# baycom/tfrec

Hardware: AMD Instinct MI355X
Metric: IQ MSamples/s through demod+decode (batched streams) (higher is better)
Workload: dtype int32+f32+f64

## Files before the change

include/tfrec_amd.h:

```cpp
#ifndef TFREC_AMD_H
#define TFREC_AMD_H

#include <stddef.h>
#include <stdint.h>

#ifdef __cplusplus
extern "C" {
#endif

#define TFREC_AMD_BLOCK_BYTES 65536
#define TFREC_AMD_FIFO_DEPTH 4
#define TFREC_AMD_BLOCK_BYTES_10X 655360
#define TFREC_AMD_BLOCK_DEC 8192
#define TFREC_AMD_NSLOTS 5

enum { TFREC_AMD_SLOT_TFA1 = 0, TFREC_AMD_SLOT_TFA2 = 1, TFREC_AMD_SLOT_TFA3 = 2, TFREC_AMD_SLOT_TX22 = 3,
       TFREC_AMD_SLOT_WHB = 4 };

enum {
	TFREC_AMD_OK = 0,
	TFREC_AMD_E_INVAL = -1,
	TFREC_AMD_E_NOMEM = -2,
	TFREC_AMD_E_HIP = -3,
	TFREC_AMD_E_OVERFLOW = -4,
// ... 263 lines not shown
	uint64_t floor;
	uint32_t n_hit;
	uint32_t n_frames;
} tfrec_amd_occupancy;
int tfrec_amd_enable_occupancy(tfrec_amd_ctx *ctx, uint32_t ratio, uint32_t rel);
int tfrec_amd_read_occupancy(tfrec_amd_ctx *ctx, int32_t row, tfrec_amd_occupancy *recs, uint32_t *bitmap, size_t cap_records,
			     int *n_records);

int tfrec_amd_rssi_db(int slot, int64_t rssi_raw);

int tfrec_amd_read_stage0(tfrec_amd_ctx *ctx, int stream, int16_t *out, size_t n_pairs);
int tfrec_amd_read_decimated(tfrec_amd_ctx *ctx, int stream, int16_t *out, size_t n_pairs);
typedef struct {
	uint64_t resolved;
	uint64_t host_verified;
	uint64_t host_mismatch;
	uint64_t undecidable;
	uint64_t reserved[4];
} tfrec_amd_fm_stats;
int tfrec_amd_get_fm_stats(tfrec_amd_ctx *ctx, tfrec_amd_fm_stats *out);
int tfrec_amd_atan_uncertain(tfrec_amd_ctx *ctx, uint64_t *n);
int tfrec_amd_fm_dev_probe(int device, int kind, const void *records, size_t n, int32_t *out, tfrec_amd_fm_stats *stats);
int tfrec_amd_iir_probe(int device, double cutoff, int form, const double *in, size_t n, double *out);
int tfrec_amd_read_biquad_row(tfrec_amd_ctx *ctx, int slot, int stream, int32_t *out, size_t cap_values, uint32_t *n_slots);
int tfrec_amd_get_timings(tfrec_amd_ctx *ctx, tfrec_amd_timings *out);
typedef struct {
	uint64_t biquad_segments;
	uint64_t biquad_unconverged;
	uint64_t biquad_serial;
	uint64_t tfa2_resliced;
	uint64_t tfa1_recomputed;
	uint64_t biquad_repair_slots;
	uint64_t whb_respeculated;
	uint64_t tfa1_scalar_groups;
	uint64_t tfa2_scalar_groups;
	uint64_t tfa1_vector_groups;
	uint64_t tfa2_vector_groups;
} tfrec_amd_stats;
int tfrec_amd_get_stats(tfrec_amd_ctx *ctx, tfrec_amd_stats *out);
int tfrec_amd_get_layout(tfrec_amd_ctx *ctx, int *n_streams);
int tfrec_amd_get_memory(tfrec_amd_ctx *ctx, uint64_t *device_bytes, uint64_t *pinned_host_bytes);
int tfrec_amd_read_thresh(tfrec_amd_ctx *ctx, int stream, int *thresh);

#ifdef __cplusplus
}
#endif
// ... 2 lines not shown
```

tfrec_amd/api.py:

```python
from __future__ import annotations

import ctypes as C
import os
from fractions import Fraction

import numpy as np

from . import _build
from .burst import BURST_DTYPE
from .capture import RUN_DTYPE
from .clock import CLOCK_DTYPE
from .envelope import ENVELOPE_DTYPE
from .levels import LEVEL_DTYPE
from .occupancy import OCC_DTYPE
from .sync import SYNC_DTYPE
from .track import TRACK_DTYPE

BLOCK_BYTES = 65536
BLOCK_DEC = 8192
NSLOTS = 5
FIFO_DEPTH = 4
SLOT_NAMES = ("TFA_1", "TFA_2", "TFA_3", "TX22", "WHB")

F_ALL_FLUSHES = 1
# ... 64 lines not shown
    ]
)
assert EVENT_DTYPE.itemsize == 96

EXPORTS = (
    "tfrec_amd_version", "tfrec_amd_strerror", "tfrec_amd_last_error", "tfrec_amd_create", "tfrec_amd_destroy",
    "tfrec_amd_submit_device", "tfrec_amd_submit_host", "tfrec_amd_sync", "tfrec_amd_drain_events",
    "tfrec_amd_pending_events", "tfrec_amd_rssi_db", "tfrec_amd_read_decimated", "tfrec_amd_atan_uncertain",
    "tfrec_amd_get_timings", "tfrec_amd_read_thresh", "tfrec_amd_get_stats", "tfrec_amd_get_layout", "tfrec_amd_host_alloc",
    "tfrec_amd_host_free", "tfrec_amd_read_stage0", "tfrec_amd_get_fm_stats", "tfrec_amd_fm_dev_probe",
    "tfrec_amd_fifo_depth", "tfrec_amd_get_memory", "tfrec_amd_iir_probe", "tfrec_amd_reset_streams",
    "tfrec_amd_configure_streams", "tfrec_amd_get_stream_config", "tfrec_amd_tune_streams", "tfrec_amd_get_stream_tune",
    "tfrec_amd_map_streams", "tfrec_amd_get_stream_input", "tfrec_amd_tune_streams_wide", "tfrec_amd_get_stream_tune_wide",
    "tfrec_amd_create_rate", "tfrec_amd_get_input_rate", "tfrec_amd_input_bytes", "tfrec_amd_resample_taps",
    "tfrec_amd_tune_streams_input", "tfrec_amd_get_stream_tune_input", "tfrec_amd_create_format", "tfrec_amd_get_input_format",
    "tfrec_amd_read_levels", "tfrec_amd_enable_capture", "tfrec_amd_read_captures", "tfrec_amd_enable_spectrum",
    "tfrec_amd_read_spectrum", "tfrec_amd_enable_occupancy", "tfrec_amd_read_occupancy", "tfrec_amd_create_dc", "tfrec_amd_get_dc",
    "tfrec_amd_read_dc", "tfrec_amd_reset_dc_rows", "tfrec_amd_create_iq", "tfrec_amd_get_iq", "tfrec_amd_read_iq", "tfrec_amd_reset_iq_rows", "tfrec_amd_create_decimated", "tfrec_amd_enable_capture_pre",
    "tfrec_amd_read_capture_pre", "tfrec_amd_enable_runs_input", "tfrec_amd_submit_runs", "tfrec_amd_read_biquad_row",
    "tfrec_amd_enable_burst_meter", "tfrec_amd_read_bursts", "tfrec_amd_stream_state_bytes", "tfrec_amd_save_streams",
    "tfrec_amd_load_streams", "tfrec_amd_enable_burst_envelope", "tfrec_amd_read_burst_envelopes",
    "tfrec_amd_enable_burst_clock", "tfrec_amd_read_burst_clocks",
    "tfrec_amd_enable_burst_track", "tfrec_amd_set_burst_track_centre", "tfrec_amd_read_burst_tracks",
    "tfrec_amd_enable_burst_sync", "tfrec_amd_read_burst_syncs",
)

_libs = {}


def library_path(experiments: bool = False, short_segments: bool = False) -> str:
    return _build.VARIANTS[_build.variant_name(experiments, short_segments)][0]


def load_library(build: bool = True, experiments: bool = False, short_segments: bool = False):
    key = _build.variant_name(experiments, short_segments)
    if key in _libs:
        return _libs[key]
    if build:
        try:
            _build.build_device_lib(experiments=bool(experiments), short_segments=bool(short_segments))
        except (OSError, FileNotFoundError):
            pass
    lib_so = library_path(experiments, short_segments)
    if key == "experiments":
        lib_so = os.environ.get("TFREC_AMD_LIB", lib_so)
    if not os.path.exists(lib_so):
        raise RuntimeError("HIP extension %s is missing: run __graft_entry__.build()" % lib_so)
# ... 7 lines not shown
    L.tfrec_amd_strerror.argtypes = [C.c_int]
    L.tfrec_amd_last_error.restype = C.c_char_p
    L.tfrec_amd_create.argtypes = [C.POINTER(Config), C.POINTER(C.c_void_p)]
    L.tfrec_amd_destroy.argtypes = [C.c_void_p]
    L.tfrec_amd_submit_device.argtypes = [C.c_void_p, C.c_void_p, C.c_size_t, C.c_int, C.c_void_p]
    L.tfrec_amd_submit_host.argtypes = [C.c_void_p, C.c_void_p, C.c_size_t, C.c_int]
    L.tfrec_amd_sync.argtypes = [C.c_void_p]
    L.tfrec_amd_drain_events.argtypes = [C.c_void_p, C.c_void_p, C.c_int, C.POINTER(C.c_int)]
    L.tfrec_amd_pending_events.argtypes = [C.c_void_p, C.POINTER(C.c_int)]
    L.tfrec_amd_rssi_db.argtypes = [C.c_int, C.c_int64]
    L.tfrec_amd_rssi_db.restype = C.c_int
    L.tfrec_amd_read_decimated.argtypes = [C.c_void_p, C.c_int, C.c_void_p, C.c_size_t]
    L.tfrec_amd_read_stage0.argtypes = [C.c_void_p, C.c_int, C.c_void_p, C.c_size_t]
    L.tfrec_amd_read_biquad_row.argtypes = [C.c_void_p, C.c_int, C.c_int, C.c_void_p, C.c_size_t, C.POINTER(C.c_uint32)]
    L.tfrec_amd_atan_uncertain.argtypes = [C.c_void_p, C.POINTER(C.c_uint64)]
    L.tfrec_amd_get_timings.argtypes = [C.c_void_p, C.POINTER(Timings)]
    L.tfrec_amd_read_thresh.argtypes = [C.c_void_p, C.c_int, C.POINTER(C.c_int)]
    L.tfrec_amd_get_stats.argtypes = [C.c_void_p, C.POINTER(Stats)]
    L.tfrec_amd_get_layout.argtypes = [C.c_void_p, C.POINTER(C.c_int)]
    L.tfrec_amd_get_memory.argtypes = [C.c_void_p, C.POINTER(C.c_uint64), C.POINTER(C.c_uint64)]
    L.tfrec_amd_get_fm_stats.argtypes = [C.c_void_p, C.POINTER(FmStats)]
    L.tfrec_amd_fm_dev_probe.argtypes = [C.c_int, C.c_int, C.c_void_p, C.c_size_t, C.c_void_p, C.POINTER(FmStats)]
    L.tfrec_amd_iir_probe.argtypes = [C.c_int, C.c_double, C.c_int, C.c_void_p, C.c_size_t, C.c_void_p]
    L.tfrec_amd_reset_streams.argtypes = [C.c_void_p, C.c_void_p, C.c_int]
    L.tfrec_amd_configure_streams.argtypes = [C.c_void_p, C.c_void_p, C.c_void_p, C.c_int]
    L.tfrec_amd_get_stream_config.argtypes = [C.c_void_p, C.c_int, C.POINTER(StreamConfig)]
    L.tfrec_amd_tune_streams.argtypes = [C.c_void_p, C.c_void_p, C.c_void_p, C.c_int]
    L.tfrec_amd_get_stream_tune.argtypes = [C.c_void_p, C.c_int, C.POINTER(C.c_int32)]
    L.tfrec_amd_map_streams.argtypes = [C.c_void_p, C.c_void_p, C.c_void_p, C.c_int]
    L.tfrec_amd_get_stream_input.argtypes = [C.c_void_p, C.c_int, C.POINTER(C.c_int32)]
    L.tfrec_amd_tune_streams_wide.argtypes = [C.c_void_p, C.c_void_p, C.c_void_p, C.c_int]
    L.tfrec_amd_get_stream_tune_wide.argtypes = [C.c_void_p, C.c_int, C.POINTER(C.c_int32)]
    L.tfrec_amd_tune_streams_input.argtypes = [C.c_void_p, C.c_void_p, C.c_void_p, C.c_int]
    L.tfrec_amd_get_stream_tune_input.argtypes = [C.c_void_p, C.c_int, C.POINTER(C.c_int32)]
    L.tfrec_amd_create_rate.argtypes = [C.POINTER(Config), C.c_int32, C.c_int32, C.POINTER(C.c_void_p)]
    L.tfrec_amd_get_input_rate.argtypes = [C.c_void_p, C.POINTER(C.c_int32), C.POINTER(C.c_int32)]
    L.tfrec_amd_input_bytes.argtypes = [C.c_void_p, C.c_int, C.POINTER(C.c_size_t)]
    L.tfrec_amd_resample_taps.argtypes = [C.c_int32, C.c_int32, C.c_void_p, C.c_int, C.POINTER(C.c_int)]
    L.tfrec_amd_create_format.argtypes = [C.POINTER(Config), C.c_int32, C.c_int32, C.c_int32, C.POINTER(C.c_void_p)]
    L.tfrec_amd_get_input_format.argtypes = [C.c_void_p, C.POINTER(C.c_int32)]
    L.tfrec_amd_read_levels.argtypes = [C.c_void_p, C.c_void_p, C.c_size_t, C.POINTER(C.c_int)]
    L.tfrec_amd_enable_capture.argtypes = [C.c_void_p, C.c_uint32, C.c_uint64]
    L.tfrec_amd_read_captures.argtypes = [C.c_void_p, C.c_void_p, C.c_size_t, C.POINTER(C.c_uint32), C.c_void_p, C.c_size_t,
                                          C.POINTER(C.c_uint64)]
    L.tfrec_amd_enable_spectrum.argtypes = [C.c_void_p, C.c_int32, C.c_int32, C.c_int32]
    L.tfrec_amd_read_spectrum.argtypes = [C.c_void_p, C.c_int32, C.c_void_p, C.c_void_p, C.c_size_t, C.c_void_p, C.POINTER(C.c_int)]
# ... 575 lines not shown

    def stats(self) -> dict:
        st = Stats()
        _check(self.L, self.L.tfrec_amd_get_stats(self.h, C.byref(st)))
        return {n: int(getattr(st, n)) for n, _ in Stats._fields_}


def fm_dev_nrzs_probe(records: np.ndarray, device: int = 0) -> np.ndarray:
    L = load_library()
    q = np.ascontiguousarray(records, dtype=np.int32).reshape(-1, 4)
    out = np.empty(len(q), dtype=np.int32)
    _check(L, L.tfrec_amd_fm_dev_probe(device, 2, q.ctypes.data, len(q), out.ctypes.data, None))
    return out


def iir_probe(cutoff: float, x: np.ndarray, form: int = 1, device: int = 0) -> np.ndarray:
    L = load_library()
    xin = np.ascontiguousarray(x, dtype=np.float64)
    out = np.empty(len(xin), dtype=np.float64)
    _check(L, L.tfrec_amd_iir_probe(device, float(cutoff), int(form), xin.ctypes.data, len(xin), out.ctypes.data))
    return out


def fm_dev_probe(records: np.ndarray, device: int = 0, cross: bool = False):
    L = load_library()
    q = (np.ascontiguousarray(records, dtype=np.int64).reshape(-1, 2) if cross
         else np.ascontiguousarray(records, dtype=np.int32).reshape(-1, 4))
    out = np.empty(len(q), dtype=np.int32)
    st = FmStats()
    _check(L, L.tfrec_amd_fm_dev_probe(device, 1 if cross else 0, q.ctypes.data, len(q), out.ctypes.data, C.byref(st)))
    return out, {n: int(getattr(st, n)) for n, _ in FmStats._fields_[:4]}


def events_canon(events: np.ndarray):
    L = load_library()
    events = events[events["status"] != STATUS_BITS]
    m = np.empty((len(events), 71), dtype=np.int64)
    m[:, 0] = events["slot"]
    m[:, 1] = events["end_sample"]
    m[:, 2] = events["byte_cnt"]
    slots = events["slot"].tolist()
    raws = events["rssi_raw"].tolist()
    m[:, 3] = [L.tfrec_amd_rssi_db(sl, rw) for sl, rw in zip(slots, raws)]
    m[:, 4] = events["offset"]
    m[:, 5:69] = events["rdata"]
    m[:, 69] = events["rssi_raw"]
# ... 39 lines not shown
```

tfrec_amd/csrc/capi_create.h:

```cpp
#pragma once

static BiquadCoef biquad_coef(double cutoff)
{
	static const struct {
		double cutoff, b0, a1, a2;
	} known[] = {
		{ 0.5 / (384000.0 / 17240), 0x1.27f98b1037a14p-8, 0x1.cd1527f4a26e2p+0, -0x1.a36a1c41c6995p-1 },
		{ 0.5 / (384000.0 / 9600), 0x1.7ed02b18a270dp-10, 0x1.e397ac010fc89p+0, -0x1.ca2cf85850d62p-1 },
		{ 0.5 / (384000.0 / 8842), 0x1.461fa1a309718p-10, 0x1.e5d4f47377e30p+0, -0x1.ce36282a35d90p-1 },
		{ 2.0 / 64.0, 0x1.14a67102a1ffdp-7, 0x1.b949652fa3970p+0, -0x1.83dd316f714e0p-1 },
		{ 0.0025 / 64.0, 0x1.02ae4cfc8910ap-26, 0x1.ffe9409fe171bp+0, -0x1.ffd283451f7d3p-1 },
	};
	BiquadCoef c;
	for (const auto &k : known)
		if (k.cutoff == cutoff) {
			c.b0 = k.b0;
			c.b1 = k.b0 + k.b0;
			c.b2 = k.b0;
			c.a1 = k.a1;
			c.a2 = k.a2;
			return c;
		}
	const double i = 1.0 / tan(cutoff * M_PI);
	const double s = sqrt(2.0);
// ... 511 lines not shown
		TRY(own_device(c, c->lev.d_records[k], n * (size_t)c->cfg.max_blocks * sizeof(tfrec_amd_level)));
	return make_side_lane(c, c->lev.lane);
}

static int make_streams(tfrec_amd_ctx *c, PipeCtl &S)
{
	int prio_lo = 0, prio_hi = 0;
	(void)hipDeviceGetStreamPriorityRange(&prio_lo, &prio_hi);
	hipStream_t cp = nullptr;
	TRY(own_stream(c, S.fs, prio_hi));
	TRY(own_stream(c, cp, 0));
	TRY(own_stream(c, S.cs, prio_hi));
	S.ws = S.fs;
	c->cpy = cp;
	if (c->cfg.flags & TFREC_AMD_F_SERIAL_CHAINS)
		return TFREC_AMD_OK;
	TRY(own_stream(c, S.t1, prio_hi));
	TRY(own_stream(c, S.aux, prio_hi));
	const char *dp = TFREC_KNOB_STR("DEEP");
	c->deep = dp ? atoi(dp) != 0 : true;
	c->fmdev_k2 = has_kind(c->launch, 1) && has_kind(c->launch, 2);
	S.k2 = S.cs;
	S.kw = S.aux;
	S.vx = S.aux;
	if (!c->deep)
		return TFREC_AMD_OK;
	TRY(own_stream(c, S.k2, 0));
	TRY(own_stream(c, S.kw, 0));
	S.ws = S.kw;
	if (c->fmdev_k2) {
		TRY(own_stream(c, S.fq, prio_lo));
		TRY(own_stream(c, S.ks, prio_lo));
	}
	TRY(own_stream(c, c->cpy, prio_lo));
	S.vx = cp;
	return TFREC_AMD_OK;
}

static int make_pipes(tfrec_amd_ctx *c, const PipeCtl &S)
{
	const bool serial = (c->cfg.flags & TFREC_AMD_F_SERIAL_CHAINS) != 0;
	const bool timing = (c->cfg.flags & TFREC_AMD_F_TIMING) != 0;
	for (int k = 0; k < kSets; k++) {
		PipeCtl &P = c->pipe[k];
		P = S;
		for (hipEvent_t *e : { &P.done[0], &P.done[1], &P.done[2], &P.ev_win, &P.ev_fork, &P.ev_k2, &P.ev_kw, &P.ev_fm,
				       &P.ev_spec, &c->ev_in[k], &P.ev_front, &c->copied[k] })
			TRY(own_event(c, *e, hipEventDisableTiming));
		if (!serial)
			TRY(own_event(c, P.ev_aux, hipEventDisableTiming));
		if (timing) {
			for (hipEvent_t &e : c->ev[k])
				TRY(own_event(c, e, hipEventDefault));
			if (!serial) {
				for (hipEvent_t &e : c->tev[k])
					TRY(own_event(c, e, hipEventDefault));
				P.tev = c->tev[k];
			}
		}
		P.whb_carry = c->d_whbcarry;
		P.fmdev_wmax = c->fmdev_k2 ? c->wmax : 0;
		P.fm_flag_eps = c->fm_flag_eps;
	}
	return TFREC_AMD_OK;
}

static int init_context(tfrec_amd_ctx *c)
{
	if (const char *fe = TFREC_KNOB_STR("FM_FLAG_EPS"))
		c->fm_flag_eps = std::max(1e-9, atof(fe));
	if (const char *cg = TFREC_KNOB_STR("COPY_GUESS_MIN"))
		c->copy_guess = c->copy_guess_min = (uint32_t)std::max(1, atoi(cg));
	TRY(register_chains(c));
// ... 157 lines not shown
```

tfrec_amd/csrc/capi_probe.h:

```cpp
#pragma once

static void account_fm_log(FmTotals *t, const EventBuf &eb)
{
	t->resolved += eb.uncertain;
	t->undecidable += eb.fm_undecidable;
	const uint32_t n = std::min<uint32_t>(eb.fm_logged, (uint32_t)kFmLogCap);
	const double scale = 16384.0 * (1.0 / M_PI);
	for (uint32_t k = 0; k < n; k++) {
		const int want = d2i_host(atan2(eb.fm_log[k].cj, eb.fm_log[k].cr) * scale);
		t->verified++;
		if (want != eb.fm_log[k].result)
			t->mismatch++;
	}
}

static void report_debug_stats(tfrec_amd_ctx *c, int set, int n_blocks)
{
#ifdef TFREC_AMD_VECSTAT
	if (c->submit_seq == 3) {
		(void)hipDeviceSynchronize();
		unsigned long long st[16] = { 0 };
		(void)hipMemcpy(st, c->win[set].stats, sizeof(st), hipMemcpyDeviceToHost);
		fprintf(stderr, "VECSTAT (one submit) TFA_1: groups %llu, stale piece %llu, entered-with-none hazard %llu, > 64 bits in a lane %llu, lanes with 32 ones or more %llu; TFA_2 family: groups %llu, entered with relative 0 %llu, > 16 rounds %llu, > 64 bits in a lane %llu, walks of the groups that converged %llu\n", st[8], st[9], st[10], st[11], st[5], st[12], st[13], st[14], st[15], st[6]);
	}
// ... 199 lines not shown
		stats->undecidable = tmp.undecidable;
	}
	return rc;
}

int tfrec_amd_iir_probe(int device, double cutoff, int form, const double *in, size_t n, double *out)
{
	if (!in || !out || n == 0 || n > (1u << 24) || form < 0 || form > 1 || !(cutoff > 0.0 && cutoff < 0.5))
		return TFREC_AMD_E_INVAL;
	HIPCHK(hipSetDevice(device));
	double *d_in = nullptr, *d_out = nullptr;
	int rc = TFREC_AMD_OK;
	if (hipMalloc((void **)&d_in, n * 8) != hipSuccess || hipMalloc((void **)&d_out, n * 8) != hipSuccess)
		rc = TFREC_AMD_E_NOMEM;
	if (rc == TFREC_AMD_OK && (hipMemcpy(d_in, in, n * 8, hipMemcpyHostToDevice) != hipSuccess ||
				   launch_iir_probe(nullptr, d_in, n, biquad_coef(cutoff), d_out, form) != hipSuccess ||
				   hipMemcpy(out, d_out, n * 8, hipMemcpyDeviceToHost) != hipSuccess))
		rc = hip_fail(hipGetLastError(), "iir_probe");
	(void)hipFree(d_in);
	(void)hipFree(d_out);
	return rc;
}

int tfrec_amd_read_thresh(tfrec_amd_ctx *c, int stream, int *thresh)
{
	if (!c || !thresh || stream < 0 || stream >= c->cfg.n_streams)
		return TFREC_AMD_E_INVAL;
	if (!c->settings.per_stream && c->cfg.thresh) {
		*thresh = c->cfg.thresh;
		return TFREC_AMD_OK;
	}
	TRY(tfrec_amd_sync(c));
	FskState f;
	HIPCHK(hipMemcpy(&f, c->d_fsk + stream, sizeof(f), hipMemcpyDeviceToHost));
	*thresh = f.thresh;
	return TFREC_AMD_OK;
}

int tfrec_amd_get_timings(tfrec_amd_ctx *c, tfrec_amd_timings *out)
{
	if (!c || !out)
		return TFREC_AMD_E_INVAL;
	if (!c->timed)
		return TFREC_AMD_E_STATE;
	const int set = c->last_drained >= 0 ? c->last_drained : c->head;
	hipEvent_t *ev = c->ev[set], *tev = c->tev[set];
// ... 109 lines not shown
```

tfrec_amd/csrc/chains2.hip:

```cpp
#include <stdlib.h>

#include <algorithm>

#include "decoder_dev.h"
#include "launch.h"
#include <type_traits>
#include "whb_chain_asm.h"

namespace tfrec {

constexpr int kSpecLbi = -(1 << 30);

__device__ __forceinline__ int whb_hook_perturb(const WinTables &T)
{
#ifdef TFREC_AMD_EXPERIMENTS
	return T.whb_test_perturb;
#else
	return 0;
#endif
}
__device__ __forceinline__ int whb_hook_force_fail(const WinTables &T)
{
#ifdef TFREC_AMD_EXPERIMENTS
	return T.whb_force_fail;
// ... 158 lines not shown
				const dim3 wgrid(n_streams), wblock(64);
				const int wlds = 64 * 64;
				if (flags & TFREC_AMD_F_BITS) {
					hipLaunchKernelGGL((whb_demod_kernel<true, false>), wgrid, wblock, wlds, P.aux, dec, dec_stride, dev32, n_streams,
							   n_blocks, sample_base, L, a, T, events, eb, flags);
				} else {
					hipLaunchKernelGGL((whb_demod_kernel<false, false>), wgrid, wblock, wlds, P.aux, dec, dec_stride, dev32, n_streams,
							   n_blocks, sample_base, L, a, T, events, eb, flags);
					whb_spec = a;
				}
				mark(kMarkWhbDemodEnd, P.aux);
				mark(kMarkWhbDecodeEnd, P.aux);
				mark(kMarkWhbCommitEnd, P.aux);
			}
	}
	if (whb_spec >= 0) {
		if (P.vx != P.aux) {
			TRY(hipEventRecord(P.ev_aux, P.aux));
			TRY(hipStreamWaitEvent(P.vx, P.ev_aux, 0));
		}
		mark(kMarkWhbCheck, P.vx);
		hipLaunchKernelGGL(whb_chain_kernel, dim3((n_streams + kChkStreams - 1) / kChkStreams), dim3(64 * (1 + kChkProducers)), kChkLdsBytes,
				   P.vx, n_streams, L, whb_spec, T);
		hipLaunchKernelGGL(whb_check_kernel, dim3(n_streams), block, 0, P.vx, n_streams, L, whb_spec, T, P.whb_carry);
		ChainLaunch Lr = L;
		WinTables Tr = T;
		Tr.whbpub = L.states[whb_spec];
		Lr.states[whb_spec] = T.whbscr;
		hipLaunchKernelGGL((whb_demod_kernel<true, true>), dim3((n_streams + 63) / 64), block, 64 * 64, P.vx, dec, dec_stride, dev32, n_streams,
				   n_blocks, sample_base, Lr, whb_spec, Tr, events, eb, flags);
		mark(kMarkWhbCheckEnd, P.vx);
		TRY(hipEventRecord(P.done[1], P.vx));
	} else {
		TRY(hipEventRecord(P.done[1], P.aux));
	}
	static_assert(kMarkTfa2End == kMarkTfa2Coop + 3 && kMarkTfa1End == kMarkTfa1Coop + 3, "a slicer chain's marks are consecutive");
	auto slicer_chain = [&](int kind, hipStream_t s_, int m0) {
		if (kind == 0)
			hipLaunchKernelGGL(mark_kernel, dim3(std::max(1, win_blocks / 16)), dim3(256), 0, s_, dec, dec_stride, n_streams,
					   n_blocks, L, T);
		const size_t slds = (kind == 0 ? 8 : 4) * 64 * sizeof(uint4);
		hipLaunchKernelGGL(slicer_kernel, dim3(std::max(64, win_blocks)), block, slds, s_, dec, dec_stride, ld16, n_streams, n_blocks, L, T,
				   lanes, head_chunks, kind, 0);
		mark(m0, s_);
		hipLaunchKernelGGL(coop_slicer_kernel, dim3(coop_blocks), block, 0, s_, dec, dec_stride, ld16, n_streams, n_blocks, L,
				   T, kind);
		mark(m0 + 1, s_);
		hipLaunchKernelGGL(decode_kernel, dim3(dec_blocks), block, 0, s_, n_streams, L, T, kind);
		mark(m0 + 2, s_);
		hipLaunchKernelGGL(commit_kernel, grid, block, 0, s_, dec, dec_stride, ld16, n_streams, n_blocks, sample_base, L, T,
				   events, eb, flags, lanes, kind);
		if (kind == 1)
			hipLaunchKernelGGL(commit_wave_kernel, dim3(256), block, 0, s_, dec, dec_stride, ld16, n_streams, n_blocks,
					   sample_base, L, T, events, eb, flags);
		mark(m0 + 3, s_);
// ... 40 lines not shown
		TRY(hipEventRecord(P.ev_k2, P.k2));
		TRY(hipStreamWaitEvent(P.cs, P.ev_k2, 0));
		mark(kMarkTfa2Slicer, P.cs);
		slicer_chain(1, P.cs, kMarkTfa2Coop);
	}
	TRY(hipEventRecord(P.done[0], P.cs));
	if (has_tfa1) {
		if (!has_tfa2)
			TRY(hipStreamWaitEvent(P.t1, P.ev_win, 0));
		mark(kMarkTfa1Slicer, P.t1);
		slicer_chain(0, P.t1, kMarkTfa1Coop);
	}
	TRY(hipEventRecord(P.done[2], P.t1));
#undef TRY
	return hipGetLastError();
}

hipError_t whb_chain_lds_optin()
{
	return hipFuncSetAttribute(reinterpret_cast<const void *>(&whb_chain_kernel), hipFuncAttributeMaxDynamicSharedMemorySize,
				   (int)kChkLdsBytes);
}

}
```

tfrec_amd/csrc/launch.h:

```cpp
#pragma once

namespace tfrec {

struct FrontOut {
	uint32_t *dec;             size_t dec_stride;
	unsigned long long *mask;  size_t mask_stride;
	uint32_t *prevdec;
	int16_t *fmdev;            size_t fmdev_stride;
	int n_streams, n_blocks;
};
struct History {
	const uint8_t *in;
	uint8_t *out;
};
struct RateTable {
	int p, q, t;
	const float *taps;
};
struct CaptureBufs {
	CaptureState *state;
	CaptureStage *stage;
	int stage_cap;
	uint2 *cnt;
	uint4 *base;
// ... 45 lines not shown
			   const FrontTapsCfg &taps, bool in16, const uint2 *tune, const uint4 *chan);
hipError_t launch_decin(hipStream_t st, const uint8_t *in, size_t stride, const uint4 *chan, const FrontOut &o, uint32_t *last, int thresh,
			const StreamCfg *scfg);
hipError_t launch_decin_runs(hipStream_t st, const RunsTables &r, const FrontOut &o, uint32_t *last, int thresh, const StreamCfg *scfg);
hipError_t launch_fmdev(hipStream_t st, const FrontOut &o, EventBuf *eb, int wmax, double flag_eps);
hipError_t launch_levels(hipStream_t st, const FrontOut &o, LevelState *lev, const StreamCfg *scfg, tfrec_amd_level *out);
hipError_t launch_capture(hipStream_t st, const FrontOut &o, long long sample_base, const CaptureBufs &b, const StreamCfg *scfg);
hipError_t launch_capture_pre(hipStream_t st, const FrontOut &o, long long sample_base, const CaptureBufs &b, uint32_t *pre);
hipError_t launch_burst_meter(hipStream_t st, const FrontOut &o, const CaptureBufs &b, tfrec_amd_burst *out);
hipError_t launch_burst_envelope(hipStream_t st, const FrontOut &o, const CaptureBufs &b, tfrec_amd_envelope *out);
hipError_t launch_burst_clock(hipStream_t st, const FrontOut &o, const CaptureBufs &b, tfrec_amd_clock *out);
hipError_t launch_burst_track(hipStream_t st, const FrontOut &o, const CaptureBufs &b, const TrackBufs &k);
hipError_t launch_burst_sync(hipStream_t st, const FrontOut &o, const CaptureBufs &b, const SyncBufs &k);
hipError_t launch_spectrum(hipStream_t st, int fmt, const uint8_t *iq, size_t stride, const SpectrumBufs &b);
hipError_t launch_occupancy(hipStream_t st, const SpectrumBufs &b, uint32_t ratio, uint32_t rel, tfrec_amd_occupancy *recs, uint32_t *bits);
hipError_t launch_fm_probe(hipStream_t st, const int32_t *quads, size_t n, int32_t *out, EventBuf *eb, int kind);
hipError_t launch_iir_probe(hipStream_t st, const double *in, size_t n, const BiquadCoef &c, double *out, int form);
hipError_t launch_chains(hipStream_t st, const FrontOut &o, long long sample_base, const ChainLaunch &L, tfrec_amd_event *events,
			 EventBuf *eb, uint32_t flags);
hipError_t launch_threshold(hipStream_t st, const FrontOut &o, FskState *fsk, int wmax, const StreamCfg *scfg);
hipError_t launch_pipeline(const PipeCtl &P, const FrontOut &o, long long sample_base, const ChainLaunch &L, const WinTables &T, int16_t *ld16,
			   int32_t *dev32, tfrec_amd_event *events, EventBuf *eb, uint32_t flags);
hipError_t whb_chain_lds_optin();
struct StateTable;
hipError_t launch_stream_state(hipStream_t st, bool load, const StateTable &T, const int32_t *list, int n_list, uint8_t *stage);

}
```

tfrec_amd/csrc/tfrec_dev.h:

```cpp
#pragma once

#include <hip/hip_runtime.h>
#include <stddef.h>
#include <stdint.h>

#include "../../include/tfrec_amd.h"

#if defined(__HIP_DEVICE_COMPILE__)
#if !defined(__gfx950__)
#error "tfrec_amd: the device code targets gfx950 (MI355X) only"
#endif
#if defined(__AMDGCN_WAVEFRONT_SIZE) && __AMDGCN_WAVEFRONT_SIZE != 64
#error "tfrec_amd: the device code assumes 64-lane wavefronts"
#endif
#endif

namespace tfrec {

constexpr int kBlockDec = TFREC_AMD_BLOCK_DEC;
constexpr int kIndexSpan = 2 * kBlockDec;
constexpr int kTailBytes = 112;
constexpr int kNSlots = TFREC_AMD_NSLOTS;
constexpr int kFmtU8 = TFREC_AMD_FMT_U8, kFmtS8 = TFREC_AMD_FMT_S8, kFmtS16 = TFREC_AMD_FMT_S16, kFmtF32 = TFREC_AMD_FMT_F32;
constexpr int kFmtDec16 = TFREC_AMD_FMT_DEC16;
// ... 291 lines not shown
	int32_t *whbdense;
	int32_t whbdense_stride;
	int32_t *whbdense_n;
	unsigned long long *whbxbits;
	double2 *whbxsnap;
	int32_t whbx_stride;
	int32_t whb_force_fail;
	int32_t whb_submit_seq;
	ChainState *whbscr;
	ChainState *whbpub;
	int32_t whb_test_perturb;
	int32_t tfa2_vec;
	int32_t tfa1_vec;
};
constexpr int kStatusDead = 0xff;

struct PipeCtl {
	hipStream_t fs;
	hipStream_t ws;
	hipEvent_t ev_front;
	hipStream_t k2, kw;
	hipStream_t cs, aux, t1;
	hipStream_t vx;
	hipEvent_t ev_aux;
	int *whb_carry;
	hipEvent_t ev_win;
	hipEvent_t ev_fork;
	hipEvent_t ev_k2, ev_kw;
	hipEvent_t ev_fm;
	hipStream_t fq;
	hipStream_t ks;
	hipEvent_t ev_spec;
	hipEvent_t done[3];
	hipEvent_t *tev;
	int fmdev_wmax;
	double fm_flag_eps;
};
enum TimingMark : int {
	kMarkWindows = 0,
	kMarkTfa2Spec = 1, kMarkTfa2Repair = 2, kMarkTfa2Fix = 3, kMarkTfa2BiquadEnd = 4,
	kMarkTfa2Coop = 5, kMarkTfa2Decode = 6, kMarkTfa2Commit = 7, kMarkTfa2End = 8,
	kMarkWhbSpec = 9, kMarkWhbRepair = 10, kMarkWhbFix = 11, kMarkWhbBiquadEnd = 12,
	kMarkWhbDemodEnd = 13, kMarkWhbDecodeEnd = 14, kMarkWhbCommitEnd = 15,
	kMarkTfa1Slicer = 16, kMarkTfa1Coop = 17, kMarkTfa1Decode = 18, kMarkTfa1Commit = 19, kMarkTfa1End = 20,
	kMarkWindowsEnd = 21, kMarkWhbDemod = 22, kMarkTfa2Slicer = 23, kMarkFmdev = 24, kMarkFmdevEnd = 25,
	kMarkWhbCheck = 26, kMarkWhbCheckEnd = 27,
	kTimingMarks = 28
// ... 27 lines not shown
```

tfrec_amd/csrc/whb_check.h:

```cpp
#pragma once

#ifndef TFREC_AMD_CHK_STREAMS
#define TFREC_AMD_CHK_STREAMS 32
#endif
constexpr int kChkStreams = TFREC_AMD_CHK_STREAMS;
constexpr int kChkProducers = 2;
constexpr int kChkPerProducer = kChkStreams / kChkProducers;
static_assert(kChkStreams <= 64 && kChkStreams % kChkProducers == 0, "a lane per stream, the streams split evenly");
constexpr int kChkPairRow = 64 * 4 + 4;
constexpr int kChkDevRow = 64 + 4;
struct ChkBuf {
	uint32_t pair[kChkStreams * kChkPairRow];
	uint32_t dev[kChkStreams * kChkDevRow];
};
constexpr size_t kChkLdsBytes = 2 * sizeof(ChkBuf);

__global__ __launch_bounds__(64 * (1 + kChkProducers)) void whb_chain_kernel(int n_streams, ChainLaunch L, int a, WinTables T)
{
	extern __shared__ __attribute__((aligned(16))) uint8_t chk_lds[];
	ChkBuf *const buf = reinterpret_cast<ChkBuf *>(chk_lds);
	const int wave = (int)threadIdx.x >> 6, ln = (int)threadIdx.x & 63;
	const int s0 = (int)blockIdx.x * kChkStreams;
	const ChainParams &p = L.params[a];
	const double a1 = p.iir_avg.a1, a2 = p.iir_avg.a2, bh = 0.5 * p.iir_avg.b0;
	const int my_s = s0 + ln;
	const bool my_on = ln < kChkStreams && my_s < n_streams;
	const int my_rounds = my_on ? T.whbdense_n[my_s] >> 6 : 0;
	int rmax = my_rounds;
#pragma unroll
	for (int o = 32; o >= 1; o >>= 1) {
		const int other = __shfl_xor(rmax, o, 64);
		rmax = other > rmax ? other : rmax;
	}
	rmax = __builtin_amdgcn_readfirstlane(rmax);
	if (rmax == 0)
		return;
	if (wave == 0) {
		double y1 = 0.0, y2 = 0.0;
		if (my_on) {
			const WhbExact st = T.whbx[my_s];
			y1 = st.y1;
			y2 = st.y2;
		}
		unsigned long long *const xbits = T.whbxbits + (size_t)(my_on ? my_s : 0) * T.whbx_stride;
		double2 *const xsnap = T.whbxsnap + (size_t)(my_on ? my_s : 0) * T.whbx_stride;
		__syncthreads();
		for (int r = 0; r < rmax; r++) {
			if (r < my_rounds) {
				const ChkBuf &b = buf[r & 1];
				const double2 *prow = reinterpret_cast<const double2 *>(b.pair + ln * kChkPairRow);
				const uint4 *drow = reinterpret_cast<const uint4 *>(b.dev + ln * kChkDevRow);
				uint32_t acc[2] = { 0u, 0u };
				double2 pq[2][8];
				uint4 dq[2][2];
				auto fetch = [&](int h, int g8) {
#pragma unroll
					for (int j = 0; j < 8; j++)
						pq[h][j] = prow[8 * g8 + j];
					dq[h][0] = drow[2 * g8];
					dq[h][1] = drow[2 * g8 + 1];
				};
				fetch(0, 0);
#pragma unroll
				for (int g8 = 0; g8 < 8; g8++) {
					const int h = g8 & 1;
					if (g8 + 1 < 8)
						fetch(h ^ 1, g8 + 1);
					const int dv[8] = { (int)dq[h][0].x, (int)dq[h][0].y, (int)dq[h][0].z, (int)dq[h][0].w,
							    (int)dq[h][1].x, (int)dq[h][1].y, (int)dq[h][1].z, (int)dq[h][1].w };
#pragma unroll
					for (int j = 0; j < 8; j++) {
						const double P = pq[h][j].x, B2 = pq[h][j].y;
						const double y = ((B2 + a1 * y1) + P) + a2 * y2;
						y2 = y1;
						y1 = y;
						const int yi = (int)y;
						asm("v_cmp_lt_i32 vcc, %1, %2\n\tv_addc_co_u32 %0, vcc, %0, %0, vcc" : "+v"(acc[g8 >> 2]) : "v"(dv[j]), "v"(yi) : "vcc");
					}
				}
				xbits[r] = (unsigned long long)__brev(acc[0]) | ((unsigned long long)__brev(acc[1]) << 32);
				xsnap[r] = make_double2(y1, y2);
			}
			__syncthreads();
		}
	} else {
		const int q0 = (wave - 1) * kChkPerProducer;
		int rounds[kChkPerProducer], h1[kChkPerProducer], h2[kChkPerProducer];
		const int32_t *row[kChkPerProducer];
#pragma unroll
		for (int q = 0; q < kChkPerProducer; q++) {
			const int s = s0 + q0 + q;
			const bool on = s < n_streams;
			rounds[q] = __builtin_amdgcn_readlane(my_rounds, (q0 + q) & 63);
			row[q] = T.whbdense + (size_t)(on ? s : 0) * T.whbdense_stride;
			const WhbExact st = T.whbx[on ? s : 0];
			h1[q] = __builtin_amdgcn_readfirstlane(st.fd1);
			h2[q] = __builtin_amdgcn_readfirstlane(st.fd2);
		}
		int cur[kChkPerProducer], nxt[kChkPerProducer];
#pragma unroll
		for (int q = 0; q < kChkPerProducer; q++) {
			cur[q] = rounds[q] > 0 ? row[q][ln] : 0;
			nxt[q] = rounds[q] > 1 ? row[q][64 + ln] : 0;
		}
		auto lay_out = [&](ChkBuf &b, int r) {
#pragma unroll
			for (int q = 0; q < kChkPerProducer; q++) {
				if (r < rounds[q]) {
					const int d0 = cur[q];
					const int s1 = __builtin_amdgcn_update_dpp(0, d0, 0x138, 0xf, 0xf, false);
					const int d1 = ln == 0 ? h1[q] : s1;
					const int s2 = __builtin_amdgcn_update_dpp(0, d1, 0x138, 0xf, 0xf, false);
					const int d2 = ln == 0 ? h2[q] : s2;
					const double t0 = bh * (double)d0, t1 = bh * (double)d1, t2 = bh * (double)d2;
					const double P = __builtin_fma(2.0, t1, t0);
					*reinterpret_cast<double2 *>(b.pair + (q0 + q) * kChkPairRow + 4 * ln) = make_double2(P, t2);
					b.dev[(q0 + q) * kChkDevRow + ln] = (uint32_t)d0;
					h1[q] = __builtin_amdgcn_readlane(d0, 63);
					h2[q] = __builtin_amdgcn_readlane(d0, 62);
				}
			}
		};
		lay_out(buf[0], 0);
		__syncthreads();
		for (int r = 0; r < rmax; r++) {
			int far[kChkPerProducer];
#pragma unroll
			for (int q = 0; q < kChkPerProducer; q++)
				far[q] = r + 2 < rounds[q] ? row[q][64 * (r + 2) + ln] : 0;
#pragma unroll
			for (int q = 0; q < kChkPerProducer; q++)
				cur[q] = nxt[q];
			if (r + 1 < rmax)
				lay_out(buf[(r + 1) & 1], r + 1);
#pragma unroll
			for (int q = 0; q < kChkPerProducer; q++)
				nxt[q] = far[q];
			__syncthreads();
		}
	}
}

constexpr int kChkLockCap = 256;
__global__ __launch_bounds__(64) void whb_check_kernel(int n_streams, ChainLaunch L, int a, WinTables T, int *__restrict__ carry_io)
{
	__shared__ int lk_pos[kChkLockCap], lk_avgf[kChkLockCap];
	__shared__ uint32_t lk_meta[kChkLockCap];
	const int s = (int)blockIdx.x, ln = (int)threadIdx.x;
	if (s >= n_streams)
		return;
	const ChainParams &p = L.params[a];
	const double a1 = p.iir_avg.a1, a2 = p.iir_avg.a2, bh = 0.5 * p.iir_avg.b0;
	const int N = T.whbdense_n[s], R = N >> 6;
	const int32_t *dense = T.whbdense + (size_t)s * T.whbdense_stride;
	const unsigned long long *xbits = T.whbxbits + (size_t)s * T.whbx_stride;
	const double2 *xsnap = T.whbxsnap + (size_t)s * T.whbx_stride;
	const WhbExact st0 = T.whbx[s];
	const int tp_ = whb_hook_perturb(T);
	const int tol = tp_ > 1 ? tp_ : (tp_ < -1 ? -tp_ : 1);
	auto input = [&](int pos) -> int { return pos >= 0 ? dense[pos] : (pos == -1 ? st0.fd1 : st0.fd2); };
	auto run = [&](int rr, int cnt, double &y1, double &y2, unsigned long long &bits) {
		const int p0 = 64 * rr;
		if (rr == 0) {
			y1 = st0.y1;
			y2 = st0.y2;
		} else {
			const double2 sn = xsnap[rr - 1];
			y1 = sn.x;
			y2 = sn.y;
		}
		double t1 = bh * (double)input(p0 - 1), t2 = bh * (double)input(p0 - 2);
		bits = 0ull;
		for (int k = 0; k < cnt; k++) {
			const int d = dense[p0 + k];
			const double t0 = bh * (double)d;
			const double P = __builtin_fma(2.0, t1, t0);
			const double y = ((t2 + a1 * y1) + P) + a2 * y2;
			bits |= (unsigned long long)(d < (int)y ? 1u : 0u) << k;
			y2 = y1;
			y1 = y;
			t2 = t1;
			t1 = t0;
		}
	};
	double yf1 = 0.0, yf2 = 0.0;
	unsigned long long tailbits = 0ull;
	if (ln == 0)
		run(R, N & 63, yf1, yf2, tailbits);
	tailbits = __shfl(tailbits, 0, 64);
	auto word = [&](int i) -> unsigned long long { return i < R ? xbits[i] : (i == R ? tailbits : 0ull); };
	const uint4 *recrow = reinterpret_cast<const uint4 *>(T.whbrec + (size_t)s * T.whbrec_stride);
	int carry = carry_io[s];
	const int carry_in = carry;
	bool bad = false;
	int cbase = 0, nlocks = 0;
	bool ended = false;
	int last_delta = 0;
	bool have_last = false, last_closed = false;
	auto do_locks = [&]() {
		for (int b0 = 0; b0 < nlocks; b0 += 64) {
			const int i = b0 + ln;
			const bool on = i < nlocks;
			double y1 = 0.0, y2 = 0.0;
			unsigned long long bits;
			const int pos = on ? lk_pos[i] : 0;
			run(pos >> 6, on ? (pos & 63) + 1 : 0, y1, y2, bits);
			const uint32_t meta = on ? lk_meta[i] : 0u;
			const int delta = (int)y1 - (on ? lk_avgf[i] : 0);
			const bool b = on && (delta > tol || delta < -tol || (delta != 0 && (meta & kWhbRecAmb)));
			bad = bad || __ballot(b) != 0ull;
			const int nb = nlocks - b0 < 64 ? nlocks - b0 : 64;
			last_delta = __shfl(delta, nb - 1, 64);
			last_closed = (__shfl((int)meta, nb - 1, 64) & (int)kWhbRecClosed) != 0;
// ... 38 lines not shown
		}
		carry = __shfl(carry, 0, 64);
		const bool lock = normal && (meta & kWhbRecLock) != 0u;
		const unsigned long long lm = __ballot(lock);
		if (lm) {
			if (nlocks + 64 > kChkLockCap)
				do_locks();
			if (lock) {
				const int i = nlocks + __builtin_popcountll(lm & ((1ull << ln) - 1ull));
				lk_pos[i] = pos0 + nv - 1;
				lk_avgf[i] = (int)rec.w;
				lk_meta[i] = meta;
			}
			nlocks += __builtin_popcountll(lm);
			__syncthreads();
		}
	}
	if (nlocks)
		do_locks();
	bad = __ballot(bad) != 0ull || cbase != N;
	if (have_last)
		carry = last_closed ? 0 : last_delta;
	if (ln == 0) {
		WhbExact st = st0;
		st.carry = carry_in;
		st.pad_ = 0;
		T.whbx0[s] = st;
		bad = bad || T.whbseen[s] != T.whbgen[s];
		if (whb_hook_force_fail(T) > 0 && (s + T.whb_submit_seq) % whb_hook_force_fail(T) == 0)
			bad = true;
		st.y1 = yf1;
		st.y2 = yf2;
		st.fd1 = input(N - 1);
		st.fd2 = input(N - 2);
		st.carry = st.pad_ = 0;
		T.whbx[s] = st;
		carry_io[s] = bad ? 0 : carry;
		T.whbfail[s] = bad ? 1 : 0;
	}
}
```

Baseline: 305,000.

## Move WHB tail round into chain kernel and run check on separate stream

The chain kernel now also processes the partial tail round of each stream's dense input and writes the final state and the start snapshot (whbx0). This removes the serial single-lane tail recurrence from the check kernel. The check and demod kernels are launched on a new low-priority stream that waits on an event recorded after the chain kernel, so they can overlap with other work in deep mode. A standalone probe API for the chain kernel is added for testing. The risks are the extra event sync and the chain kernel no longer returning early when no stream has a full round.

```diff
diff --git a/include/tfrec_amd.h b/include/tfrec_amd.h
--- a/include/tfrec_amd.h
+++ b/include/tfrec_amd.h
@@ -309,6 +309,13 @@
 int tfrec_amd_atan_uncertain(tfrec_amd_ctx *ctx, uint64_t *n);
 int tfrec_amd_fm_dev_probe(int device, int kind, const void *records, size_t n, int32_t *out, tfrec_amd_fm_stats *stats);
 int tfrec_amd_iir_probe(int device, double cutoff, int form, const double *in, size_t n, double *out);
+typedef struct {
+	double y1, y2;
+	int32_t fd1, fd2;
+	int32_t reserved[2];
+} tfrec_amd_whb_state;
+int tfrec_amd_whb_chain_probe(int device, int n_streams, const int32_t *in, size_t stride, const int32_t *n, tfrec_amd_whb_state *state,
+			      tfrec_amd_whb_state *start, uint64_t *bits, double *snaps);
 int tfrec_amd_read_biquad_row(tfrec_amd_ctx *ctx, int slot, int stream, int32_t *out, size_t cap_values, uint32_t *n_slots);
 int tfrec_amd_get_timings(tfrec_amd_ctx *ctx, tfrec_amd_timings *out);
 typedef struct {
diff --git a/tfrec_amd/api.py b/tfrec_amd/api.py
--- a/tfrec_amd/api.py
+++ b/tfrec_amd/api.py
@@ -110,7 +110,7 @@
     "tfrec_amd_load_streams", "tfrec_amd_enable_burst_envelope", "tfrec_amd_read_burst_envelopes",
     "tfrec_amd_enable_burst_clock", "tfrec_amd_read_burst_clocks",
     "tfrec_amd_enable_burst_track", "tfrec_amd_set_burst_track_centre", "tfrec_amd_read_burst_tracks",
-    "tfrec_amd_enable_burst_sync", "tfrec_amd_read_burst_syncs",
+    "tfrec_amd_enable_burst_sync", "tfrec_amd_read_burst_syncs", "tfrec_amd_whb_chain_probe",
 )
 
 _libs = {}
@@ -164,6 +164,8 @@
     L.tfrec_amd_get_fm_stats.argtypes = [C.c_void_p, C.POINTER(FmStats)]
     L.tfrec_amd_fm_dev_probe.argtypes = [C.c_int, C.c_int, C.c_void_p, C.c_size_t, C.c_void_p, C.POINTER(FmStats)]
     L.tfrec_amd_iir_probe.argtypes = [C.c_int, C.c_double, C.c_int, C.c_void_p, C.c_size_t, C.c_void_p]
+    L.tfrec_amd_whb_chain_probe.argtypes = [C.c_int, C.c_int, C.c_void_p, C.c_size_t, C.c_void_p, C.c_void_p, C.c_void_p, C.c_void_p,
+                                            C.c_void_p]
     L.tfrec_amd_reset_streams.argtypes = [C.c_void_p, C.c_void_p, C.c_int]
     L.tfrec_amd_configure_streams.argtypes = [C.c_void_p, C.c_void_p, C.c_void_p, C.c_int]
     L.tfrec_amd_get_stream_config.argtypes = [C.c_void_p, C.c_int, C.POINTER(StreamConfig)]
@@ -785,6 +787,26 @@
     return out
 
 
+WHB_STATE_DTYPE = np.dtype([("y1", "<f8"), ("y2", "<f8"), ("fd1", "<i4"), ("fd2", "<i4"), ("reserved", "<i4", (2,))])
+assert WHB_STATE_DTYPE.itemsize == 32
+
+
+def whb_chain_probe(rows: np.ndarray, n: np.ndarray, state: np.ndarray, device: int = 0):
+    L = load_library()
+    x = np.ascontiguousarray(rows, dtype=np.int32)
+    ns, stride = x.shape
+    cnt = np.ascontiguousarray(n, dtype=np.int32)
+    end = np.array(state, dtype=WHB_STATE_DTYPE)
+    assert cnt.shape == (ns,) and end.shape == (ns,)
+    start = np.empty(ns, dtype=WHB_STATE_DTYPE)
+    words = stride // 64 + 1
+    bits = np.empty((ns, words), dtype=np.uint64)
+    snaps = np.empty((ns, words, 2), dtype=np.float64)
+    _check(L, L.tfrec_amd_whb_chain_probe(device, ns, x.ctypes.data, stride, cnt.ctypes.data, end.ctypes.data, start.ctypes.data,
+                                          bits.ctypes.data, snaps.ctypes.data))
+    return end, start, bits, snaps
+
+
 def fm_dev_probe(records: np.ndarray, device: int = 0, cross: bool = False):
     L = load_library()
     q = (np.ascontiguousarray(records, dtype=np.int64).reshape(-1, 2) if cross
diff --git a/tfrec_amd/csrc/capi_create.h b/tfrec_amd/csrc/capi_create.h
--- a/tfrec_amd/csrc/capi_create.h
+++ b/tfrec_amd/csrc/capi_create.h
@@ -557,7 +557,7 @@
 	c->fmdev_k2 = has_kind(c->launch, 1) && has_kind(c->launch, 2);
 	S.k2 = S.cs;
 	S.kw = S.aux;
-	S.vx = S.aux;
+	S.vx = S.vc = S.aux;
 	if (!c->deep)
 		return TFREC_AMD_OK;
 	TRY(own_stream(c, S.k2, 0));
@@ -569,6 +569,7 @@
 	}
 	TRY(own_stream(c, c->cpy, prio_lo));
 	S.vx = cp;
+	TRY(own_stream(c, S.vc, prio_lo));
 	return TFREC_AMD_OK;
 }
 
@@ -583,7 +584,8 @@
 				       &P.ev_spec, &c->ev_in[k], &P.ev_front, &c->copied[k] })
 			TRY(own_event(c, *e, hipEventDisableTiming));
 		if (!serial)
-			TRY(own_event(c, P.ev_aux, hipEventDisableTiming));
+			for (hipEvent_t *e : { &P.ev_aux, &P.ev_chain })
+				TRY(own_event(c, *e, hipEventDisableTiming));
 		if (timing) {
 			for (hipEvent_t &e : c->ev[k])
 				TRY(own_event(c, e, hipEventDefault));
diff --git a/tfrec_amd/csrc/capi_probe.h b/tfrec_amd/csrc/capi_probe.h
--- a/tfrec_amd/csrc/capi_probe.h
+++ b/tfrec_amd/csrc/capi_probe.h
@@ -245,6 +245,43 @@
 	return rc;
 }
 
+int tfrec_amd_whb_chain_probe(int device, int n_streams, const int32_t *in, size_t stride, const int32_t *n, tfrec_amd_whb_state *state,
+			      tfrec_amd_whb_state *start, uint64_t *bits, double *snaps)
+{
+	static_assert(sizeof(tfrec_amd_whb_state) == sizeof(WhbExact) && offsetof(tfrec_amd_whb_state, fd1) == offsetof(WhbExact, fd1),
+		      "tfrec_amd_whb_state is WhbExact");
+	if (!in || !n || !state || !start || !bits || !snaps || n_streams < 1 || n_streams > (1 << 16) || stride < 1 || stride > (1u << 24))
+		return TFREC_AMD_E_INVAL;
+	for (int s = 0; s < n_streams; s++)
+		if (n[s] < 0 || (size_t)n[s] > stride)
+			return TFREC_AMD_E_INVAL;
+	HIPCHK(hipSetDevice(device));
+	const size_t ns = (size_t)n_streams, words = stride / 64 + 1;
+	const size_t b_in = ns * stride * 4, b_n = ns * 4, b_x = ns * sizeof(WhbExact), b_bits = ns * words * 8, b_snap = ns * words * 16;
+	int32_t *d_in = nullptr, *d_n = nullptr;
+	WhbExact *d_x = nullptr, *d_x0 = nullptr;
+	unsigned long long *d_bits = nullptr;
+	double2 *d_snap = nullptr;
+	int rc = TFREC_AMD_OK;
+	if (hipMalloc((void **)&d_in, b_in) != hipSuccess || hipMalloc((void **)&d_n, b_n) != hipSuccess || hipMalloc((void **)&d_x, b_x) != hipSuccess ||
+	    hipMalloc((void **)&d_x0, b_x) != hipSuccess || hipMalloc((void **)&d_bits, b_bits) != hipSuccess ||
+	    hipMalloc((void **)&d_snap, b_snap) != hipSuccess)
+		rc = TFREC_AMD_E_NOMEM;
+	const WhbChainProbe b = { .n_streams = n_streams, .avg = biquad_coef(0.0025 / 64.0), .dense = d_in, .dense_stride = (int)stride, .dense_n = d_n,
+				  .x = d_x, .x0 = d_x0, .xbits = d_bits, .xsnap = d_snap, .x_stride = (int)words };
+	if (rc == TFREC_AMD_OK && (hipMemcpy(d_in, in, b_in, hipMemcpyHostToDevice) != hipSuccess || hipMemcpy(d_n, n, b_n, hipMemcpyHostToDevice) != hipSuccess ||
+				   hipMemcpy(d_x, state, b_x, hipMemcpyHostToDevice) != hipSuccess || hipMemset(d_x0, 0xff, b_x) != hipSuccess ||
+				   hipMemset(d_bits, 0, b_bits) != hipSuccess || hipMemset(d_snap, 0, b_snap) != hipSuccess ||
+				   launch_whb_chain_probe(nullptr, b) != hipSuccess || hipMemcpy(state, d_x, b_x, hipMemcpyDeviceToHost) != hipSuccess ||
+				   hipMemcpy(start, d_x0, b_x, hipMemcpyDeviceToHost) != hipSuccess ||
+				   hipMemcpy(bits, d_bits, b_bits, hipMemcpyDeviceToHost) != hipSuccess ||
+				   hipMemcpy(snaps, d_snap, b_snap, hipMemcpyDeviceToHost) != hipSuccess))
+		rc = hip_fail(hipGetLastError(), "whb_chain_probe");
+	for (void *p : { (void *)d_in, (void *)d_n, (void *)d_x, (void *)d_x0, (void *)d_bits, (void *)d_snap })
+		(void)hipFree(p);
+	return rc;
+}
+
 int tfrec_amd_read_thresh(tfrec_amd_ctx *c, int stream, int *thresh)
 {
 	if (!c || !thresh || stream < 0 || stream >= c->cfg.n_streams)
diff --git a/tfrec_amd/csrc/chains2.hip b/tfrec_amd/csrc/chains2.hip
--- a/tfrec_amd/csrc/chains2.hip
+++ b/tfrec_amd/csrc/chains2.hip
@@ -204,15 +204,19 @@
 		mark(kMarkWhbCheck, P.vx);
 		hipLaunchKernelGGL(whb_chain_kernel, dim3((n_streams + kChkStreams - 1) / kChkStreams), dim3(64 * (1 + kChkProducers)), kChkLdsBytes,
 				   P.vx, n_streams, L, whb_spec, T);
-		hipLaunchKernelGGL(whb_check_kernel, dim3(n_streams), block, 0, P.vx, n_streams, L, whb_spec, T, P.whb_carry);
+		if (P.vc != P.vx) {
+			TRY(hipEventRecord(P.ev_chain, P.vx));
+			TRY(hipStreamWaitEvent(P.vc, P.ev_chain, 0));
+		}
+		hipLaunchKernelGGL(whb_check_kernel, dim3(n_streams), block, 0, P.vc, n_streams, L, whb_spec, T, P.whb_carry);
 		ChainLaunch Lr = L;
 		WinTables Tr = T;
 		Tr.whbpub = L.states[whb_spec];
 		Lr.states[whb_spec] = T.whbscr;
-		hipLaunchKernelGGL((whb_demod_kernel<true, true>), dim3((n_streams + 63) / 64), block, 64 * 64, P.vx, dec, dec_stride, dev32, n_streams,
+		hipLaunchKernelGGL((whb_demod_kernel<true, true>), dim3((n_streams + 63) / 64), block, 64 * 64, P.vc, dec, dec_stride, dev32, n_streams,
 				   n_blocks, sample_base, Lr, whb_spec, Tr, events, eb, flags);
-		mark(kMarkWhbCheckEnd, P.vx);
-		TRY(hipEventRecord(P.done[1], P.vx));
+		mark(kMarkWhbCheckEnd, P.vc);
+		TRY(hipEventRecord(P.done[1], P.vc));
 	} else {
 		TRY(hipEventRecord(P.done[1], P.aux));
 	}
@@ -299,4 +303,27 @@
 				   (int)kChkLdsBytes);
 }
 
-}
+hipError_t launch_whb_chain_probe(hipStream_t st, const WhbChainProbe &b)
+{
+	hipError_t e = whb_chain_lds_optin();
+	if (e != hipSuccess)
+		return e;
+	ChainLaunch L = {};
+	L.n_active = 1;
+	L.params[0].kind = 2;
+	L.params[0].iir_avg = b.avg;
+	WinTables T = {};
+	T.whbdense = const_cast<int32_t *>(b.dense);
+	T.whbdense_stride = b.dense_stride;
+	T.whbdense_n = const_cast<int32_t *>(b.dense_n);
+	T.whbx = b.x;
+	T.whbx0 = b.x0;
+	T.whbxbits = b.xbits;
+	T.whbxsnap = b.xsnap;
+	T.whbx_stride = b.x_stride;
+	hipLaunchKernelGGL(whb_chain_kernel, dim3((b.n_streams + kChkStreams - 1) / kChkStreams), dim3(64 * (1 + kChkProducers)), kChkLdsBytes, st,
+			   b.n_streams, L, 0, T);
+	return hipGetLastError();
+}
+
+}
diff --git a/tfrec_amd/csrc/launch.h b/tfrec_amd/csrc/launch.h
--- a/tfrec_amd/csrc/launch.h
+++ b/tfrec_amd/csrc/launch.h
@@ -91,6 +91,18 @@
 hipError_t launch_pipeline(const PipeCtl &P, const FrontOut &o, long long sample_base, const ChainLaunch &L, const WinTables &T, int16_t *ld16,
 			   int32_t *dev32, tfrec_amd_event *events, EventBuf *eb, uint32_t flags);
 hipError_t whb_chain_lds_optin();
+struct WhbChainProbe {
+	int n_streams;
+	BiquadCoef avg;
+	const int32_t *dense;
+	int dense_stride;
+	const int32_t *dense_n;
+	WhbExact *x, *x0;
+	unsigned long long *xbits;
+	double2 *xsnap;
+	int x_stride;
+};
+hipError_t launch_whb_chain_probe(hipStream_t st, const WhbChainProbe &b);
 struct StateTable;
 hipError_t launch_stream_state(hipStream_t st, bool load, const StateTable &T, const int32_t *list, int n_list, uint8_t *stage);
 
diff --git a/tfrec_amd/csrc/tfrec_dev.h b/tfrec_amd/csrc/tfrec_dev.h
--- a/tfrec_amd/csrc/tfrec_dev.h
+++ b/tfrec_amd/csrc/tfrec_dev.h
@@ -337,7 +337,9 @@
 	hipStream_t k2, kw;
 	hipStream_t cs, aux, t1;
 	hipStream_t vx;
+	hipStream_t vc;
 	hipEvent_t ev_aux;
+	hipEvent_t ev_chain;
 	int *whb_carry;
 	hipEvent_t ev_win;
 	hipEvent_t ev_fork;
diff --git a/tfrec_amd/csrc/whb_check.h b/tfrec_amd/csrc/whb_check.h
--- a/tfrec_amd/csrc/whb_check.h
+++ b/tfrec_amd/csrc/whb_check.h
@@ -25,7 +25,8 @@
 	const double a1 = p.iir_avg.a1, a2 = p.iir_avg.a2, bh = 0.5 * p.iir_avg.b0;
 	const int my_s = s0 + ln;
 	const bool my_on = ln < kChkStreams && my_s < n_streams;
-	const int my_rounds = my_on ? T.whbdense_n[my_s] >> 6 : 0;
+	const int my_n = my_on ? T.whbdense_n[my_s] : 0;
+	const int my_rounds = my_n >> 6, my_tail = my_n & 63;
 	int rmax = my_rounds;
 #pragma unroll
 	for (int o = 32; o >= 1; o >>= 1) {
@@ -33,14 +34,17 @@
 		rmax = other > rmax ? other : rmax;
 	}
 	rmax = __builtin_amdgcn_readfirstlane(rmax);
-	if (rmax == 0)
-		return;
 	if (wave == 0) {
 		double y1 = 0.0, y2 = 0.0;
+		int fd1 = 0, fd2 = 0;
 		if (my_on) {
-			const WhbExact st = T.whbx[my_s];
+			WhbExact st = T.whbx[my_s];
 			y1 = st.y1;
 			y2 = st.y2;
+			fd1 = st.fd1;
+			fd2 = st.fd2;
+			st.carry = st.pad_ = 0;
+			T.whbx0[my_s] = st;
 		}
 		unsigned long long *const xbits = T.whbxbits + (size_t)(my_on ? my_s : 0) * T.whbx_stride;
 		double2 *const xsnap = T.whbxsnap + (size_t)(my_on ? my_s : 0) * T.whbx_stride;
@@ -83,6 +87,35 @@
 			}
 			__syncthreads();
 		}
+		__syncthreads();
+		{
+			const ChkBuf &b = buf[rmax & 1];
+			const int lr = ln < kChkStreams ? ln : 0;
+			const double2 *prow = reinterpret_cast<const double2 *>(b.pair + lr * kChkPairRow);
+			const uint32_t *drow = b.dev + lr * kChkDevRow;
+			unsigned long long bits = 0ull;
+#pragma unroll 8
+			for (int j = 0; j < 64; j++) {
+				const double2 pb = prow[j];
+				const double y = ((pb.y + a1 * y1) + pb.x) + a2 * y2;
+				const bool take = j < my_tail;
+				const bool below = (int)drow[j] < (int)y;
+				y2 = take ? y1 : y2;
+				y1 = take ? y : y1;
+				bits |= (unsigned long long)(take && below ? 1u : 0u) << j;
+			}
+			if (my_on) {
+				xbits[my_rounds] = bits;
+				const int32_t *dense = T.whbdense + (size_t)my_s * T.whbdense_stride;
+				WhbExact st;
+				st.y1 = y1;
+				st.y2 = y2;
+				st.fd1 = my_n >= 1 ? dense[my_n - 1] : fd1;
+				st.fd2 = my_n >= 2 ? dense[my_n - 2] : (my_n == 1 ? fd1 : fd2);
+				st.carry = st.pad_ = 0;
+				T.whbx[my_s] = st;
+			}
+		}
 	} else {
 		const int q0 = (wave - 1) * kChkPerProducer;
 		int rounds[kChkPerProducer], h1[kChkPerProducer], h2[kChkPerProducer];
@@ -103,10 +136,10 @@
 			cur[q] = rounds[q] > 0 ? row[q][ln] : 0;
 			nxt[q] = rounds[q] > 1 ? row[q][64 + ln] : 0;
 		}
-		auto lay_out = [&](ChkBuf &b, int r) {
+		auto lay_out = [&](ChkBuf &b, int r, bool tail = false) {
 #pragma unroll
 			for (int q = 0; q < kChkPerProducer; q++) {
-				if (r < rounds[q]) {
+				if (tail || r < rounds[q]) {
 					const int d0 = cur[q];
 					const int s1 = __builtin_amdgcn_update_dpp(0, d0, 0x138, 0xf, 0xf, false);
 					const int d1 = ln == 0 ? h1[q] : s1;
@@ -138,6 +171,13 @@
 				nxt[q] = far[q];
 			__syncthreads();
 		}
+#pragma unroll
+		for (int q = 0; q < kChkPerProducer; q++) {
+			const int nt = __builtin_amdgcn_readlane(my_tail, (q0 + q) & 63);
+			cur[q] = ln < nt ? row[q][64 * rounds[q] + ln] : 0;
+		}
+		lay_out(buf[rmax & 1], rmax, true);
+		__syncthreads();
 	}
 }
 
@@ -155,7 +195,7 @@
 	const int32_t *dense = T.whbdense + (size_t)s * T.whbdense_stride;
 	const unsigned long long *xbits = T.whbxbits + (size_t)s * T.whbx_stride;
 	const double2 *xsnap = T.whbxsnap + (size_t)s * T.whbx_stride;
-	const WhbExact st0 = T.whbx[s];
+	const WhbExact st0 = T.whbx0[s];
 	const int tp_ = whb_hook_perturb(T);
 	const int tol = tp_ > 1 ? tp_ : (tp_ < -1 ? -tp_ : 1);
 	auto input = [&](int pos) -> int { return pos >= 0 ? dense[pos] : (pos == -1 ? st0.fd1 : st0.fd2); };
@@ -183,12 +223,7 @@
 			t1 = t0;
 		}
 	};
-	double yf1 = 0.0, yf2 = 0.0;
-	unsigned long long tailbits = 0ull;
-	if (ln == 0)
-		run(R, N & 63, yf1, yf2, tailbits);
-	tailbits = __shfl(tailbits, 0, 64);
-	auto word = [&](int i) -> unsigned long long { return i < R ? xbits[i] : (i == R ? tailbits : 0ull); };
+	auto word = [&](int i) -> unsigned long long { return i <= R ? xbits[i] : 0ull; };
 	const uint4 *recrow = reinterpret_cast<const uint4 *>(T.whbrec + (size_t)s * T.whbrec_stride);
 	int carry = carry_io[s];
 	const int carry_in = carry;
@@ -273,19 +308,10 @@
 	if (have_last)
 		carry = last_closed ? 0 : last_delta;
 	if (ln == 0) {
-		WhbExact st = st0;
-		st.carry = carry_in;
-		st.pad_ = 0;
-		T.whbx0[s] = st;
+		T.whbx0[s].carry = carry_in;
 		bad = bad || T.whbseen[s] != T.whbgen[s];
 		if (whb_hook_force_fail(T) > 0 && (s + T.whb_submit_seq) % whb_hook_force_fail(T) == 0)
 			bad = true;
-		st.y1 = yf1;
-		st.y2 = yf2;
-		st.fd1 = input(N - 1);
-		st.fd2 = input(N - 2);
-		st.carry = st.pad_ = 0;
-		T.whbx[s] = st;
 		carry_io[s] = bad ? 0 : carry;
 		T.whbfail[s] = bad ? 1 : 0;
 	}
```

Result: no change. 306,700 (median of 6 runs) (+0.6%).
